# WangChangqi98/CSS

Hardware: AMD Instinct MI355X
Metric: training images/sec at 513x513 R101-DeepLabv3+ (mix_label step, labeled+unlabeled crops consumed) (higher is better)
Workload: dtype bf16

## Files before the change

css_amd/csrc/abi.hip:

```cpp
#include "../../include/css_hip.h"
#include "launchers.h"

#include <cstdlib>
#include <cstring>
#include <mutex>
#include <new>
#include <vector>

namespace {
inline hipStream_t S(css_stream_t s) { return reinterpret_cast<hipStream_t>(s); }
inline void set_dev(int device) {
  if (device >= 0) (void)hipSetDevice(device);
}
int g_cu_count[64] = {0};
int cu_count(int device) {
  int d = device;
  if (d < 0) (void)hipGetDevice(&d);
  if (d < 0 || d >= 64) return 256;
  if (!g_cu_count[d]) {
    int v = 0;
    if (hipDeviceGetAttribute(&v, hipDeviceAttributeMultiprocessorCount, d) != hipSuccess || v <= 0) v = 256;
    g_cu_count[d] = v;
  }
  return g_cu_count[d];
// ... 117 lines not shown
int css_conv2d_forward_bnstats(const void* x, const void* w, void* y, float* stats, int Mg, int N, int H, int W, int Cin, int ldx, int Ho, int Wo,
                               int Cout, int ldy, int R, int Sk, int stride, int pad, int dil, double alg_flops, int dtype, int device,
                               css_stream_t stream) {
  set_dev(device);
  ConvArgs a = {};
  a.src = x; a.wt = w; a.dst = y; a.bias = nullptr;
  a.N = N; a.Hs = H; a.Ws = W; a.Cs = Cin; a.lds = ldx;
  a.Hd = Ho; a.Wd = Wo; a.Cd = Cout; a.ldd = ldy;
  a.R = R; a.S = Sk; a.stride = stride; a.pad = pad; a.dil = dil; a.mode = 0;
  a.M = N * Ho * Wo; a.Ktot = R * Sk * Cin;
  a.stats = stats; a.stat_Mg = Mg;
  if (!stats || Mg < 128 || a.M % Mg) return CSS_ERR_ARG;
  ConvProf cp(0, 5, alg_flops, S(stream));
  cp.hbm_bytes = short_k_bytes(a, dtype);
  cp.ws_bytes = conv1x1_bytes(a, dtype);
  cp.conv_bytes = conv_alg_bytes(a, dtype);
  return css_launch_conv(a, dtype, cu_count(device), S(stream), g_prof_on ? &cp : nullptr);
}
int css_conv2d_forward_bnstats_tile_rows(const void* x, const void* w, void* y, int N, int H, int W, int Cin, int ldx, int Ho, int Wo, int Cout,
                                         int ldy, int R, int Sk, int stride, int pad, int dil, int dtype, int device) {
  ConvArgs a = {};
  a.src = x; a.wt = w; a.dst = y; a.bias = nullptr;
  a.N = N; a.Hs = H; a.Ws = W; a.Cs = Cin; a.lds = ldx;
  a.Hd = Ho; a.Wd = Wo; a.Cd = Cout; a.ldd = ldy;
  a.R = R; a.S = Sk; a.stride = stride; a.pad = pad; a.dil = dil; a.mode = 0;
  a.M = N * Ho * Wo; a.Ktot = R * Sk * Cin;
  alignas(16) static float dummy[4];
  a.stats = dummy; a.stat_Mg = a.M;
  return css_conv_tile_rows_(a, dtype, cu_count(device));
}
int css_conv2d_dgrad(const void* dy, const void* w_t, void* dx, int N, int H, int W, int Cin, int lddx, int Ho, int Wo, int Cout, int lddy, int R,
                     int Sk, int stride, int pad, int dil, double alg_flops, int dtype, int device, css_stream_t stream) {
  set_dev(device);
  if (stride != 1 && stride != 2) return CSS_ERR_ARG;
  ConvArgs a = {};
  a.src = dy; a.wt = w_t; a.dst = dx; a.bias = nullptr;
  a.N = N; a.Hs = Ho; a.Ws = Wo; a.Cs = Cout; a.lds = lddy;
  a.Hd = H; a.Wd = W; a.Cd = Cin; a.ldd = lddx;
  a.R = R; a.S = Sk; a.stride = stride; a.pad = pad; a.dil = dil; a.mode = 1;
  a.M = N * H * W; a.Ktot = R * Sk * Cout;
  ConvProf cp(1, 6, alg_flops, S(stream));
  cp.ws_bytes = conv1x1_bytes(a, dtype);
  cp.conv_bytes = conv_alg_bytes(a, dtype);
  return css_launch_conv(a, dtype, cu_count(device), S(stream), g_prof_on ? &cp : nullptr);
}
static int dgrad_add_impl(const void* dy, const void* w_t, void* dx, const void* addend, int ld_add, const unsigned char* mask, int N, int H, int W, int Cin,
                          int lddx, int Ho, int Wo, int Cout, int lddy, int R, int Sk, int stride, int pad, int dil, double alg_flops, int dtype,
                          int device, css_stream_t stream) {
  set_dev(device);
  if (stride != 1 && stride != 2) return CSS_ERR_ARG;
  if (mask) {
    const int vec = dtype == CSS_BF16 ? 8 : 4;
    if (!addend || (Cin % vec) || (lddx % vec) || (ld_add % vec) || (reinterpret_cast<uintptr_t>(dx) & 15) || (reinterpret_cast<uintptr_t>(addend) & 15))
      return CSS_ERR_ARG;
  }
  ConvArgs a = {};
  a.src = dy; a.wt = w_t; a.dst = dx; a.bias = nullptr;
  a.N = N; a.Hs = Ho; a.Ws = Wo; a.Cs = Cout; a.lds = lddy;
  a.Hd = H; a.Wd = W; a.Cd = Cin; a.ldd = lddx;
  a.R = R; a.S = Sk; a.stride = stride; a.pad = pad; a.dil = dil; a.mode = 1; a.addend = addend; a.ld_add = ld_add; a.add_mask = mask;
  a.M = N * H * W; a.Ktot = R * Sk * Cout;
  ConvProf cp(1, 6, alg_flops, S(stream));
  cp.ws_bytes = conv1x1_bytes(a, dtype);
  cp.conv_bytes = conv_alg_bytes(a, dtype);
  return css_launch_conv(a, dtype, cu_count(device), S(stream), g_prof_on ? &cp : nullptr);
}
int css_conv2d_dgrad_add(const void* dy, const void* w_t, void* dx, const void* addend, int ld_add, int N, int H, int W, int Cin, int lddx, int Ho, int Wo, int Cout, int lddy, int R,
                     int Sk, int stride, int pad, int dil, double alg_flops, int dtype, int device, css_stream_t stream) {
  return dgrad_add_impl(dy, w_t, dx, addend, ld_add, nullptr, N, H, W, Cin, lddx, Ho, Wo, Cout, lddy, R, Sk, stride, pad, dil, alg_flops, dtype, device, stream);
}
int css_conv2d_dgrad_add_masked(const void* dy, const void* w_t, void* dx, const void* addend, int ld_add, const unsigned char* mask, int N, int H, int W, int Cin,
                                int lddx, int Ho, int Wo, int Cout, int lddy, int R, int Sk, int stride, int pad, int dil, double alg_flops, int dtype,
                                int device, css_stream_t stream) {
  if (!mask) return CSS_ERR_ARG;
  return dgrad_add_impl(dy, w_t, dx, addend, ld_add, mask, N, H, W, Cin, lddx, Ho, Wo, Cout, lddy, R, Sk, stride, pad, dil, alg_flops, dtype, device, stream);
}
size_t css_conv2d_wgrad_ws_bytes(int M, int Ktot, int Cout, int dtype, int device) {
  return css_wgrad_ws_bytes_(M, Ktot, Cout, dtype, cu_count(device));
}
int css_conv2d_wgrad(const void* x, const void* dy, float* dw, float* ws, size_t ws_bytes, int N, int H, int W, int Cin, int ldx, int Ho, int Wo,
                     int Cout, int lddy, int R, int Sk, int stride, int pad, int dil, double alg_flops, int dtype, int device,
                     css_stream_t stream) {
  set_dev(device);
  WgradArgs a;
  a.ws = ws; a.ws_bytes = ws ? ws_bytes : 0;
  a.x = x; a.dy = dy; a.dw = dw;
  a.N = N; a.Hs = H; a.Ws = W; a.Cs = Cin; a.ldx = ldx;
  a.Hd = Ho; a.Wd = Wo; a.Cd = Cout; a.ldy = lddy;
  a.R = R; a.S = Sk; a.stride = stride; a.pad = pad; a.dil = dil;
  a.M = N * Ho * Wo; a.Ktot = R * Sk * Cin; a.m_per_split = a.M;
  ConvProf cp(2, 7, alg_flops, S(stream));
  return css_launch_wgrad(a, dtype, cu_count(device), S(stream), g_prof_on ? &cp : nullptr);
}
int css_conv_ws_applies(int M, int K, int ld_src, int N, int ld_dst, int R, int Sk, int stride, int pad, int has_stats, int has_addend, int ld_add,
                        int has_bias, int dtype, int n_cu) {
  static const bool no_dma = getenv("CSS_NO_DMA_CONV") != nullptr, no_256 = getenv("CSS_NO_DMA256_CONV") != nullptr;
  if (dtype != CSS_BF16 || no_dma || no_256) return 0;
  alignas(16) static float dummy[4];
  ConvArgs a = {};
  a.N = 1; a.Hs = a.Hd = 1; a.Ws = a.Wd = M; a.M = M;
  a.Cs = K; a.lds = ld_src; a.Cd = N; a.ldd = ld_dst; a.Ktot = R * Sk * K;
  a.R = R; a.S = Sk; a.stride = stride; a.pad = pad; a.dil = 1;
  a.stats = has_stats ? dummy : nullptr;
  a.addend = has_addend ? dummy : nullptr; a.ld_add = ld_add;
  a.bias = has_bias ? dummy : nullptr;
  return css_conv_ws_supported(a, n_cu > 0 ? n_cu : 256) ? 1 : 0;
}
int css_conv_c64_applies(int N, int H, int W, int Cin, int ld_src, int Cout, int ld_dst, int R, int Sk, int stride, int pad, int dil, int has_addend,
                         int has_bias, int dtype) {
  static const bool no_dma = getenv("CSS_NO_DMA_CONV") != nullptr;
  if (no_dma) return 0;
  alignas(16) static float dummy[4];
  ConvArgs a = {};
  a.N = N; a.Hs = a.Hd = H; a.Ws = a.Wd = W; a.M = N * H * W;
  a.Cs = Cin; a.lds = ld_src; a.Cd = Cout; a.ldd = ld_dst; a.Ktot = R * Sk * Cin;
  a.R = R; a.S = Sk; a.stride = stride; a.pad = pad; a.dil = dil;
  a.src = a.wt = dummy; a.dst = dummy;
  a.addend = has_addend ? dummy : nullptr;
  a.bias = has_bias ? dummy : nullptr;
  return css_conv_c64_supported(a, dtype) ? 1 : 0;
}
int css_conv_c64_set_enabled(int on) { return css_conv_c64_set_enabled_(on); }
int css_wgrad_splits(int M, int Ktot, int Cout, int dtype, int n_cu) {
  int splits = 0, mps = 0;
  css_wgrad_plan_(M, Ktot, Cout, dtype, n_cu > 0 ? n_cu : 256, &splits, &mps);
  return splits;
}
int css_weight_layout(const float* w, void* out, int Cout, int taps, int Cin, int CinPad, int dgrad, int dtype, int device, css_stream_t stream) {
  set_dev(device);
  return css_launch_weight_layout(w, out, Cout, taps, Cin, CinPad, dgrad, dtype, S(stream));
}

int css_weight_dgrad_layout_batched(const float* flat, void* out, const long* desc, int n_layers, long total_tiles, int dtype, int device,
                                    css_stream_t stream) {
  set_dev(device);
  return css_launch_weight_dgrad_layout_batched(flat, out, desc, n_layers, total_tiles, dtype, S(stream));
}

int css_bn_nrb(int Mg, int G, int C, int dtype) { return css_bn_nrb_(Mg, G, C, dtype); }
int css_bn_stats(const void* y, int Mg, int G, int C, int ld, double* partial, int dtype, int device, css_stream_t stream) {
  set_dev(device);
  return css_launch_bn_stats(y, Mg, G, C, ld, partial, dtype, S(stream));
}
int css_bn_reduce(const double* partial, int nrb, int C, int G, double* sums, float* dgamma, float* dbeta, int accumulate, double count_local,
                  int device, css_stream_t stream) {
  set_dev(device);
  return css_launch_bn_reduce(partial, nrb, C, G, sums, dgamma, dbeta, accumulate, count_local, S(stream));
}
int css_bn_reduce_finalize(const double* partial, int nrb, int G, double count, const float* gamma, const float* beta, float* running_mean,
                           float* running_var, float momentum, float eps, float* mean, float* invstd, float* scale, float* shift, int C,
                           int device, css_stream_t stream) {
  set_dev(device);
  return css_launch_bn_reduce_finalize(partial, nrb, G, count, gamma, beta, running_mean, running_var, momentum, eps, mean, invstd, scale, shift,
                                       C, S(stream));
}
int css_bn_reduce_finalize_slabs(const float* partial, int M, int Mg, int G, double count, const float* gamma, const float* beta,
                                 float* running_mean, float* running_var, float momentum, float eps, float* mean, float* invstd, float* scale,
                                 float* shift, double* sums_out, int C, const void* y, int ldy, int tile_rows, int device, css_stream_t stream) {
  set_dev(device);
  return css_launch_bn_reduce_slabs(partial, M, Mg, G, count, gamma, beta, running_mean, running_var, momentum, eps, mean, invstd, scale, shift,
                                    sums_out, C, y, ldy, tile_rows, S(stream));
}
int css_bn_finalize(const double* sums, int G, double count, const double* count_dev, const float* gamma, const float* beta, float* running_mean,
                    float* running_var, float momentum, float eps, float* mean, float* invstd, float* scale, float* shift, int C, int device,
                    css_stream_t stream) {
  set_dev(device);
  return css_launch_bn_finalize(sums, G, count, count_dev, gamma, beta, running_mean, running_var, momentum, eps, mean, invstd, scale, shift, C, S(stream));
// ... 324 lines not shown
```

css_amd/csrc/bn.hip:

```cpp
#include "common.h"
#include <type_traits>
#include <cstdlib>

template <typename T, typename F>
__device__ __forceinline__ void channel_reduce2(F f, int Mg, int C, int rows_per_block, double* partial, bool rev = false) {
  constexpr int VEC = 16 / sizeof(T);
  const int CV = C / VEC;
  const int TPC = CV < 256 ? CV : 256;
  const int RPB = 256 / TPC;
  const int tid = threadIdx.x;
  const int cvi = tid % TPC, rg = tid / TPC;
  const int cv = blockIdx.y * TPC + cvi;
  const bool active = rg < RPB && cv < CV;
  float s0[VEC], s1[VEC];
#pragma unroll
  for (int e = 0; e < VEC; ++e) s0[e] = s1[e] = 0.f;
  const int gbase = blockIdx.z * Mg;
  const int bx = rev ? (int)(gridDim.x - 1 - blockIdx.x) : (int)blockIdx.x;
  const int row0 = gbase + bx * rows_per_block;
  const int row1 = min(gbase + Mg, row0 + rows_per_block);
  if (active) {
    int r = row0 + rg;
    for (; r + 3 * RPB < row1; r += 4 * RPB) {
      f(r, cv * VEC, s0, s1);
// ... 138 lines not shown
  shift_out[c] = bet - fmean * sc;
  if (running_mean) {
    const double unbiased = count > 1 ? var * count / (count - 1) : var;
    rm = (1.f - momentum) * rm + momentum * fmean;
    rv = (1.f - momentum) * rv + momentum * (float)unbiased;
    running_mean[c] = rm;
    running_var[c] = rv;
  }
}
__global__ __launch_bounds__(1024) void bn_reduce_kernel(const double* __restrict__ partial, int nrb, int C, int G, double* __restrict__ sums,
                                                         float* __restrict__ g1, float* __restrict__ g0, int accumulate, double count_local) {
  double t0 = 0, t1 = 0;
  if (sums && count_local > 0 && blockIdx.x == 0 && threadIdx.x < G) sums[(size_t)G * 2 * C + threadIdx.x] = count_local;
  const int ce = blockIdx.x * S2_CH + (int)threadIdx.x;
  float old0 = 0.f, old1 = 0.f;
  if (accumulate && g0 && threadIdx.x < S2_CH && ce < C) { old0 = g0[ce]; old1 = g1[ce]; }
  stage2_reduce(
      partial, C, G, [&](int g, int& lo, int& hi) { lo = g * nrb; hi = lo + nrb; },
      [&](int g, double a0, double a1, int c) {
        if (sums) { sums[(size_t)g * 2 * C + c] = a0; sums[(size_t)g * 2 * C + C + c] = a1; }
        t0 += a0; t1 += a1;
        if (g == G - 1 && g0) {
          g0[c] = old0 + (float)t0;
          g1[c] = old1 + (float)t1;
        }
      });
}
__global__ __launch_bounds__(1024) void bn_reduce_finalize_kernel(const double* __restrict__ partial, int nrb, int G, double count,
                                                                  const float* __restrict__ gamma, const float* __restrict__ beta,
                                                                  float* running_mean, float* running_var, float momentum, float eps,
                                                                  float* mean_out, float* invstd_out, float* scale_out, float* shift_out, int C) {
  const int ce = blockIdx.x * S2_CH + (int)threadIdx.x;
  float gam = 0.f, bet = 0.f, rm = 0.f, rv = 0.f;
  if (threadIdx.x < S2_CH && ce < C) {
    gam = gamma[ce]; bet = beta[ce];
    if (running_mean) { rm = running_mean[ce]; rv = running_var[ce]; }
  }
  stage2_reduce(
      partial, C, G, [&](int g, int& lo, int& hi) { lo = g * nrb; hi = lo + nrb; },
      [&](int g, double a0, double a1, int c) {
        bn_finalize_reg(a0, a1, count, gam, bet, rm, rv, running_mean, running_var, momentum, eps, mean_out + g * C, invstd_out + g * C,
                        scale_out + g * C, shift_out + g * C, c);
      });
}

__device__ __forceinline__ int slab_start(int p, int BM) { return (p >> 1) * BM + (p & 1) * (BM - 128); }
__device__ __forceinline__ int first_slab_from(int row, int BM) {
  const int t = BM == 256 ? row >> 8 : row / BM, rem = row - t * BM;
  return 2 * t + (rem == 0 ? 0 : (rem <= BM - 128 ? 1 : 2));
}
__global__ __launch_bounds__(1024) void bn_reduce_slabs_kernel(const float* __restrict__ partial, int nslab, int Mg, int G, double count,
                                                               const float* __restrict__ gamma, const float* __restrict__ beta,
                                                               float* running_mean, float* running_var, float momentum, float eps,
                                                               float* mean_out, float* invstd_out, float* scale_out, float* shift_out,
                                                               double* sums_out, int C, const bf16_t* __restrict__ y, int ldy, int BM) {
  if (sums_out && blockIdx.x == 0 && threadIdx.x < G) sums_out[(size_t)G * 2 * C + threadIdx.x] = (double)Mg;
  const int ce = blockIdx.x * S2_CH + (int)threadIdx.x;
  float gam = 0.f, bet = 0.f, rm = 0.f, rv = 0.f;
  if (!sums_out && threadIdx.x < S2_CH && ce < C) {
    gam = gamma[ce]; bet = beta[ce];
    if (running_mean) { rm = running_mean[ce]; rv = running_var[ce]; }
  }
  stage2_reduce(
      partial, C, G,
      [&](int g, int& lo, int& hi) {
        const int b = g * Mg, e = b + Mg;
        lo = first_slab_from(b, BM);
        hi = first_slab_from(e, BM);
        if (hi > nslab) hi = nslab;
      },
      [&](int g, double a0, double a1, int c) {
        if (sums_out) {
          sums_out[(size_t)g * 2 * C + c] = a0;
          sums_out[(size_t)g * 2 * C + C + c] = a1;
        } else {
          bn_finalize_reg(a0, a1, count, gam, bet, rm, rv, running_mean, running_var, momentum, eps, mean_out + g * C, invstd_out + g * C,
                          scale_out + g * C, shift_out + g * C, c);
        }
      },
      [&](int g, int c, int pl, int P, double& t0, double& t1) {
        const int b = g * Mg;
        int e = slab_start(first_slab_from(b, BM), BM);
        if (e > b + Mg) e = b + Mg;
        for (int r = b + pl; r < e; r += P) {
          const float v = (float)y[(size_t)r * ldy + c];
          t0 += (double)v;
          t1 += (double)v * (double)v;
        }
      });
}

template <typename T>
__global__ __launch_bounds__(256) void bn_stats_kernel(const T* __restrict__ y, int Mg, int C, int ld,
                                                       int rows_per_block, double* partial) {
  constexpr int VEC = 16 / sizeof(T);
  auto f = [&](int r, int c, float* s0, float* s1) {
    Vec16<T> v;
    v.load(y + (size_t)r * ld + c);
#pragma unroll
    for (int e = 0; e < VEC; ++e) {
      float x = v.f(e);
      s0[e] += x;
      s1[e] += x * x;
    }
  };
  channel_reduce2<T>(f, Mg, C, rows_per_block, partial);
}

__global__ void bn_finalize_kernel(const double* __restrict__ sums, int G, double count, const double* __restrict__ count_dev,
                                   const float* __restrict__ gamma, const float* __restrict__ beta,
                                   float* running_mean, float* running_var, float momentum, float eps,
                                   float* mean_out, float* invstd_out, float* scale_out, float* shift_out, int C) {
  int c = blockIdx.x * blockDim.x + threadIdx.x;
  if (c >= C) return;
  for (int g = 0; g < G; ++g)
    bn_finalize_one(sums[(size_t)g * 2 * C + c], sums[(size_t)g * 2 * C + C + c], count_dev ? count_dev[g] : count, gamma[c], beta[c], running_mean, running_var, momentum, eps,
                    mean_out + g * C, invstd_out + g * C, scale_out + g * C, shift_out + g * C, c);
}

__global__ void bn_eval_coeff_kernel(const float* __restrict__ gamma, const float* __restrict__ beta,
                                     const float* __restrict__ running_mean, const float* __restrict__ running_var,
                                     float eps, float* scale_out, float* shift_out, int C) {
  int c = blockIdx.x * blockDim.x + threadIdx.x;
  if (c >= C) return;
  float invstd = 1.0f / sqrtf(running_var[c] + eps);
  float sc = gamma[c] * invstd;
  scale_out[c] = sc;
  shift_out[c] = beta[c] - running_mean[c] * sc;
}

#define EW_UNROLL 4
template <typename T, bool MASK, bool RES, bool RELU>
__global__ __launch_bounds__(256) void bn_apply_kernel(const T* __restrict__ y, int ldy, const T* __restrict__ res, int ldr,
                                                       T* __restrict__ out, int ldo, const float* __restrict__ scale,
                                                       const float* __restrict__ shift, int Mg, int C, int rows_per_block,
                                                       unsigned char* __restrict__ mask, int rev) {
  constexpr int VEC = 16 / sizeof(T);
  const int CV = C / VEC;
  const int TPC = CV < 256 ? CV : 256, RPB = 256 / TPC;
  const int cvi = threadIdx.x % TPC, rg = threadIdx.x / TPC;
  const int cv = blockIdx.y * TPC + cvi;
  if (rg >= RPB || cv >= CV) return;
  const int c = cv * VEC, g = blockIdx.z;
  using P = Pairs<T>;
  f32x2 sc[P::NP], sh[P::NP];
#pragma unroll
  for (int p = 0; p < P::NP; ++p) {
    sc[p] = f32x2{scale[g * C + c + 2 * p], scale[g * C + c + 2 * p + 1]};
    sh[p] = f32x2{shift[g * C + c + 2 * p], shift[g * C + c + 2 * p + 1]};
  }
  const int gbase = g * Mg;
  const int nt = rev >> 1;
  rev &= 1;
  const int bx = rev ? (int)(gridDim.x - 1 - blockIdx.x) : (int)blockIdx.x;
  const int row0 = gbase + bx * rows_per_block, row1 = min(gbase + Mg, row0 + rows_per_block);
  for (int r = row0 + rg; r < row1; r += EW_UNROLL * RPB) {
    Vec16<T> v[EW_UNROLL], rr[EW_UNROLL];
#pragma unroll
    for (int u = 0; u < EW_UNROLL; ++u) {
      const int ru = r + u * RPB;
      if (ru < row1) {
        v[u].load(y + (size_t)ru * ldy + c, (nt & 1) != 0);
        if (RES) rr[u].load(res + (size_t)ru * ldr + c, (nt & 2) != 0);
      }
    }
#pragma unroll
    for (int u = 0; u < EW_UNROLL; ++u) {
      const int ru = r + u * RPB;
      if (ru < row1) {
        Vec16<T> o;
#pragma unroll
// ... 435 lines not shown
```

css_amd/csrc/contrast.hip:

```cpp
#include "common.h"

constexpr int CT_MAXK = 32;
struct ContrastMeta {
  int V;
  int present[CT_MAXK];
  int cntV[CT_MAXK];
  int cntH[CT_MAXK];
  int baseV[CT_MAXK];
  int baseH[CT_MAXK];
  int err;
};

__global__ __launch_bounds__(256) void contrast_classify_kernel(const float* __restrict__ label, const float* __restrict__ mask,
                                                                const float* __restrict__ prob, long sb, long sk, long sp, long psb, long psk,
                                                                long psp, int P, int HW, int K, float strong_thr, int* __restrict__ cls,
                                                                uint8_t* __restrict__ hard, ContrastMeta* meta) {
  for (int p = blockIdx.x * blockDim.x + threadIdx.x; p < P; p += gridDim.x * blockDim.x) {
    const int b = p / HW, s = p - b * HW;
    const float m = mask[p];
    int c = -1, n = 0;
    for (int k = 0; k < K; ++k) {
      const float v = label[b * sb + k * sk + s * sp] * m;
      if (v != 0.f) { if (c < 0) c = k; ++n; }
    }
    if (n > 1) atomicOr(&meta->err, 1);
    cls[p] = c;
    hard[p] = (c >= 0 && prob[b * psb + c * psk + s * psp] < strong_thr) ? 1 : 0;
  }
}

template <typename T, int C>
__global__ __launch_bounds__(256) void contrast_class_sums_kernel(const T* __restrict__ rep, int ld, const int* __restrict__ cls, int P, int K,
                                                                  int pix_per_block, float* __restrict__ out) {
  extern __shared__ float cs_lds[];
  const int tid = threadIdx.x, lane = tid & 63, wave = tid >> 6;
  float* acc = cs_lds + (size_t)wave * K * C;
  float* cnt = cs_lds + (size_t)4 * K * C + wave * CT_MAXK;
  for (int i = lane; i < K * C; i += 64) acc[i] = 0.f;
  if (lane < CT_MAXK) cnt[lane] = 0.f;
  __syncthreads();
  const int p0 = blockIdx.x * pix_per_block, p1 = min(P, p0 + pix_per_block);
  constexpr int EPL = C / 64, UN = 16;
  static_assert(EPL == 4, "a lane owns one float4 of the accumulator row");
  int cur = -1;
  float racc[4] = {0.f, 0.f, 0.f, 0.f}, rcnt = 0.f;
  auto flush = [&]() {
    if (cur >= 0) {
      float4* a4 = reinterpret_cast<float4*>(acc + cur * C + lane * EPL);
      float4 a = *a4;
      a.x += racc[0]; a.y += racc[1]; a.z += racc[2]; a.w += racc[3];
      *a4 = a;
      if (lane == 0) cnt[cur] += rcnt;
    }
    racc[0] = racc[1] = racc[2] = racc[3] = 0.f;
    rcnt = 0.f;
  };
  for (int pb = p0 + wave * 64; pb < p1; pb += 4 * 64) {
    const int ci = pb + lane < p1 ? cls[pb + lane] : -1;
#pragma unroll
    for (int u0 = 0; u0 < 64; u0 += UN) {
      int c[UN];
      float v[UN][EPL];
#pragma unroll
      for (int u = 0; u < UN; ++u) c[u] = __builtin_amdgcn_readlane(ci, u0 + u);
#pragma unroll
      for (int u = 0; u < UN; ++u) {
        if (c[u] >= 0) {
          const T* row = rep + (size_t)(pb + u0 + u) * ld + lane * EPL;
          if constexpr (sizeof(T) == 2) {
            union { uint2 u2; T e[EPL]; } pk;
            pk.u2 = *reinterpret_cast<const uint2*>(row);
#pragma unroll
            for (int e = 0; e < EPL; ++e) v[u][e] = (float)pk.e[e];
          } else {
#pragma unroll
            for (int e = 0; e < EPL; ++e) v[u][e] = (float)row[e];
          }
        }
      }
#pragma unroll
      for (int u = 0; u < UN; ++u) {
        if (c[u] < 0) continue;
        if (c[u] != cur) {
          flush();
          cur = c[u];
        }
        racc[0] += v[u][0]; racc[1] += v[u][1]; racc[2] += v[u][2]; racc[3] += v[u][3];
        rcnt += 1.f;
      }
    }
  }
  flush();
  __syncthreads();
  float* row = out + (size_t)blockIdx.x * (K * C + K);
  for (int i = tid; i < K * C; i += 256)
    row[i] = (cs_lds[i] + cs_lds[(size_t)K * C + i]) + (cs_lds[(size_t)2 * K * C + i] + cs_lds[(size_t)3 * K * C + i]);
  if (tid < K) {
    const float* cb = cs_lds + (size_t)4 * K * C;
    row[(size_t)K * C + tid] = (cb[tid] + cb[CT_MAXK + tid]) + (cb[2 * CT_MAXK + tid] + cb[3 * CT_MAXK + tid]);
  }
}
__global__ __launch_bounds__(256) void contrast_class_sums_reduce_kernel(const float* __restrict__ ws, int nrows, int n, double* __restrict__ out) {
  const int i = blockIdx.x * 256 + threadIdx.x;
  if (i >= n) return;
  double s0 = 0, s1 = 0, s2 = 0, s3 = 0;
  int r = 0;
  for (; r + 3 < nrows; r += 4) {
    s0 += (double)ws[(size_t)(r + 0) * n + i]; s1 += (double)ws[(size_t)(r + 1) * n + i];
    s2 += (double)ws[(size_t)(r + 2) * n + i]; s3 += (double)ws[(size_t)(r + 3) * n + i];
  }
  for (; r < nrows; ++r) s0 += (double)ws[(size_t)r * n + i];
  out[i] = (s0 + s1) + (s2 + s3);
}

constexpr int CHUNK_R = 16;
__global__ __launch_bounds__(256) void contrast_hist_kernel(const int* __restrict__ cls, const uint8_t* __restrict__ hard, int P, int K,
                                                            int* __restrict__ chunkhist) {
  const int lane = threadIdx.x & 63;
  const int chunk = blockIdx.x * 4 + (threadIdx.x >> 6);
  const int p0 = chunk * 64 * CHUNK_R;
  if (p0 >= P) return;
  int mine = 0;
  for (int r = 0; r < CHUNK_R; ++r) {
    const int p = p0 + r * 64 + lane;
    const int c = p < P ? cls[p] : -1;
    const int h = (p < P && c >= 0) ? hard[p] : 0;
    for (int k = 0; k < K; ++k) {
      const unsigned long long bv = __ballot(c == k), bh = __ballot(c == k && h);
      if (lane == k) mine += __popcll(bv);
      if (lane == 32 + k) mine += __popcll(bh);
    }
  }
  chunkhist[chunk * 64 + lane] = mine;
}
__global__ __launch_bounds__(64) void contrast_scan_kernel(int* __restrict__ chunkhist, int nchunks, int K, ContrastMeta* meta) {
  const int t = threadIdx.x;
  int run = 0;
  constexpr int SCAN_U = 16;
  for (int c0 = 0; c0 < nchunks; c0 += SCAN_U) {
    int v[SCAN_U];
#pragma unroll
    for (int u = 0; u < SCAN_U; ++u) v[u] = c0 + u < nchunks ? chunkhist[(c0 + u) * 64 + t] : 0;
#pragma unroll
    for (int u = 0; u < SCAN_U; ++u) {
      if (c0 + u < nchunks) chunkhist[(c0 + u) * 64 + t] = run;
      run += v[u];
    }
  }
  __shared__ int tot[64];
  tot[t] = run;
  __syncthreads();
  if (t == 0) {
    int bv = 0, bh = 0, V = 0;
    for (int k = 0; k < CT_MAXK; ++k) {
      const int cv = k < K ? tot[k] : 0, ch = k < K ? tot[32 + k] : 0;
      meta->cntV[k] = cv;
      meta->cntH[k] = ch;
      meta->baseV[k] = bv;
      meta->baseH[k] = bh;
      bv += cv;
// ... 373 lines not shown
```

css_amd/csrc/conv_wgrad.hip:

```cpp
#include "common.h"
#include "launchers.h"
#include <cstdlib>


template <typename T> struct WgFrag;
template <> struct WgFrag<bf16_t> {
  static constexpr int KS = 16;
  typedef bf16x8 frag;
  static __device__ __forceinline__ frag load(const bf16_t* tile, int RS, int kk0, int col0, int lane) {
    const int i = lane & 15, g = lane >> 4, q = i >> 2, p = i & 3;
    const bf16_t* ad = tile + (kk0 + 8 * (g >> 1) + q) * RS + col0 + 16 * (g & 1) + 4 * p;
    typedef __attribute__((address_space(3))) s16x4 lds_v4;
    s16x4 lo = __builtin_amdgcn_ds_read_tr16_b64_v4i16((lds_v4*)(ad));
    s16x4 hi = __builtin_amdgcn_ds_read_tr16_b64_v4i16((lds_v4*)(ad + 4 * RS));
    union { struct { s16x4 a, b; } s; frag f; } u;
    u.s.a = lo;
    u.s.b = hi;
    return u.f;
  }
  static __device__ __forceinline__ f32x16 mma(frag a, frag b, f32x16 c) {
    return __builtin_amdgcn_mfma_f32_32x32x16_bf16(a, b, c, 0, 0, 0);
  }
};
template <> struct WgFrag<float> {
// ... 484 lines not shown
#pragma unroll
        for (int i = 0; i < 4; ++i) acc[j][i] = __builtin_amdgcn_mfma_f32_16x16x32_bf16(j < 2 ? cur[j] : fx23[j - 2], fy[i], acc[j][i], 0, 0, 0);
#pragma unroll
      for (int g_ = 0; g_ < 16; ++g_) {
        __builtin_amdgcn_sched_group_barrier(0x008, 1, 0);
        __builtin_amdgcn_sched_group_barrier(0x006, 2, 0);
      }
      __builtin_amdgcn_sched_barrier(0);
      __builtin_amdgcn_s_barrier();
      asm volatile("" ::: "memory");
      __builtin_amdgcn_sched_barrier(0);
#pragma unroll
      for (int i = 0; i < 4; ++i) fy[i] = frag(fad[4 + i]);
      nxt[0] = frag(fad[TN + 0] + dn);
      nxt[1] = frag(fad[TN + 1] + dn);
      __builtin_amdgcn_sched_barrier(0);
      stage_half(st_i, 1, vy, vx);
      asm volatile("s_waitcnt lgkmcnt(0)" ::: "memory");
      __builtin_amdgcn_sched_barrier(0);
      __builtin_amdgcn_s_barrier();
      __builtin_amdgcn_sched_barrier(0);
      row_offsets(0, vy, vx);
#pragma unroll
      for (int k = 4; k < TN + 2; ++k) {
        fad[k] += dn;
        asm volatile("" : "+v"(fad[k]));
      }
#pragma unroll
      for (int j = 0; j < TK; ++j)
#pragma unroll
        for (int i = 0; i < 4; ++i) acc[j][4 + i] = __builtin_amdgcn_mfma_f32_16x16x32_bf16(j < 2 ? cur[j] : fx23[j - 2], fy[i], acc[j][4 + i], 0, 0, 0);
#pragma unroll
      for (int g_ = 0; g_ < 16; ++g_) {
        __builtin_amdgcn_sched_group_barrier(0x008, 1, 0);
        __builtin_amdgcn_sched_group_barrier(0x006, 2, 0);
      }
      __builtin_amdgcn_sched_barrier(0);
      __builtin_amdgcn_s_barrier();
      asm volatile("" ::: "memory");
      __builtin_amdgcn_sched_barrier(0);
      st_c = st_c == NST - 1 ? 0 : st_c + 1;
      st_i = st_i == NST - 1 ? 0 : st_i + 1;
    };
    int it = 0;
    for (; it + 1 < nit; it += 2) {
      step(fxa, fxb);
      step(fxb, fxa);
    }
    if (it < nit) step(fxa, fxb);
    WG_STAMP_END();
    if (wn == 0) __builtin_amdgcn_s_barrier();
    asm volatile("s_waitcnt vmcnt(0)" ::: "memory");
    const int l15 = lane & 15, lg = lane >> 4;
    if (a.ws) {
      float* slab = a.ws + ((size_t)t * a.splits + zz) * (256 * 256);
#pragma unroll
      for (int i = 0; i < TN; ++i) {
        const int nl = wn * WTN + i * 16 + l15;
#pragma unroll
        for (int j = 0; j < TK; ++j) {
          const int kl = wk * WTK + j * 16 + 4 * lg;
          if (a.nt & 1) __builtin_nontemporal_store(acc[j][i], reinterpret_cast<f32x4*>(slab + nl * 256 + kl));
          else *reinterpret_cast<f32x4*>(slab + nl * 256 + kl) = acc[j][i];
        }
      }
      return;
    }
#pragma unroll
    for (int i = 0; i < TN; ++i) {
      const int n = n0 + wn * WTN + i * 16 + l15;
      if (n >= a.Cd) continue;
#pragma unroll
      for (int j = 0; j < TK; ++j)
#pragma unroll
        for (int r = 0; r < 4; ++r) {
          const int k = k0 + wk * WTK + j * 16 + 4 * lg + r;
          if (k < a.Ktot) atomicAdd(a.dw + (size_t)n * a.Ktot + k, acc[j][i][r]);
        }
    }
  }
}

typedef __attribute__((ext_vector_type(4))) float wg_f32x4;
__device__ __forceinline__ float4 wg_ld4(const float4* p, bool nt) {
  if (!nt) return *p;
  const wg_f32x4 t = __builtin_nontemporal_load(reinterpret_cast<const wg_f32x4*>(p));
  return make_float4(t[0], t[1], t[2], t[3]);
}
__global__ __launch_bounds__(256) void wgrad_slab_reduce_kernel(const float* __restrict__ ws, float* __restrict__ dw, int splits, int tiles_k,
                                                                int Cd, int Ktot, int nt) {
  const int t = blockIdx.y;
  const int k0 = (t % tiles_k) * 256, n0 = (t / tiles_k) * 256;
  const int nl = blockIdx.x * 4 + (threadIdx.x >> 6), kl = (threadIdx.x & 63) * 4;
  const int n = n0 + nl, k = k0 + kl;
  if (n >= Cd || k >= Ktot) return;
  const float4* p = reinterpret_cast<const float4*>(ws + (size_t)t * splits * (256 * 256) + nl * 256 + kl);
  float4 s0 = make_float4(0.f, 0.f, 0.f, 0.f), s1 = s0, s2 = s0, s3 = s0;
  int z = 0;
  for (; z + 3 < splits; z += 4) {
    const float4 v0 = wg_ld4(p + (size_t)(z + 0) * (256 * 256 / 4), nt), v1 = wg_ld4(p + (size_t)(z + 1) * (256 * 256 / 4), nt);
    const float4 v2 = wg_ld4(p + (size_t)(z + 2) * (256 * 256 / 4), nt), v3 = wg_ld4(p + (size_t)(z + 3) * (256 * 256 / 4), nt);
    s0.x += v0.x; s0.y += v0.y; s0.z += v0.z; s0.w += v0.w;
    s1.x += v1.x; s1.y += v1.y; s1.z += v1.z; s1.w += v1.w;
    s2.x += v2.x; s2.y += v2.y; s2.z += v2.z; s2.w += v2.w;
    s3.x += v3.x; s3.y += v3.y; s3.z += v3.z; s3.w += v3.w;
  }
  for (; z < splits; ++z) {
    const float4 v0 = wg_ld4(p + (size_t)z * (256 * 256 / 4), nt);
    s0.x += v0.x; s0.y += v0.y; s0.z += v0.z; s0.w += v0.w;
  }
  const float r[4] = {(s0.x + s1.x) + (s2.x + s3.x), (s0.y + s1.y) + (s2.y + s3.y), (s0.z + s1.z) + (s2.z + s3.z), (s0.w + s1.w) + (s2.w + s3.w)};
  float* o = dw + (size_t)n * Ktot + k;
#pragma unroll
  for (int e = 0; e < 4; ++e)
    if (k + e < Ktot) o[e] += r[e];
}

template <int BN_, int BKC>
__global__ __launch_bounds__(256) void wgrad_slab_reduce_gen_kernel(const float* __restrict__ ws, float* __restrict__ dw, int splits, int tiles_k,
                                                                    int Cd, int Ktot, int nt) {
  constexpr int TPR = BKC / 4, RPB = 256 / TPR;
  const int t = blockIdx.y;
  const int k0 = (t % tiles_k) * BKC, n0 = (t / tiles_k) * BN_;
  const int nl = blockIdx.x * RPB + threadIdx.x / TPR, kl = (threadIdx.x % TPR) * 4;
  const int n = n0 + nl, k = k0 + kl;
  if (nl >= BN_ || n >= Cd || k >= Ktot) return;
  const float4* p = reinterpret_cast<const float4*>(ws + (size_t)t * splits * (BN_ * BKC) + nl * BKC + kl);
  constexpr size_t SL = (size_t)BN_ * BKC / 4;
  float4 s0 = make_float4(0.f, 0.f, 0.f, 0.f), s1 = s0, s2 = s0, s3 = s0;
  int z = 0;
  for (; z + 3 < splits; z += 4) {
    const float4 v0 = wg_ld4(p + (size_t)(z + 0) * SL, nt), v1 = wg_ld4(p + (size_t)(z + 1) * SL, nt), v2 = wg_ld4(p + (size_t)(z + 2) * SL, nt),
                 v3 = wg_ld4(p + (size_t)(z + 3) * SL, nt);
    s0.x += v0.x; s0.y += v0.y; s0.z += v0.z; s0.w += v0.w;
    s1.x += v1.x; s1.y += v1.y; s1.z += v1.z; s1.w += v1.w;
    s2.x += v2.x; s2.y += v2.y; s2.z += v2.z; s2.w += v2.w;
    s3.x += v3.x; s3.y += v3.y; s3.z += v3.z; s3.w += v3.w;
  }
  for (; z < splits; ++z) {
    const float4 v0 = wg_ld4(p + (size_t)z * SL, nt);
    s0.x += v0.x; s0.y += v0.y; s0.z += v0.z; s0.w += v0.w;
  }
  const float r[4] = {(s0.x + s1.x) + (s2.x + s3.x), (s0.y + s1.y) + (s2.y + s3.y), (s0.z + s1.z) + (s2.z + s3.z), (s0.w + s1.w) + (s2.w + s3.w)};
  float* o = dw + (size_t)n * Ktot + k;
#pragma unroll
  for (int e = 0; e < 4; ++e)
    if (k + e < Ktot) o[e] += r[e];
}


static bool wgrad_n64(int dtype, int Cd, bool big) {
  static const bool on = getenv("CSS_WGRAD_N64") && atoi(getenv("CSS_WGRAD_N64")) != 0;
  return on && dtype == CSS_BF16 && !big && Cd <= 64;
}
void css_wgrad_plan_(int M, int Ktot, int Cd, int dtype, int n_cu, int* splits_out, int* mps_out) {
  static const bool no_256 = getenv("CSS_NO_DMA256_WGRAD") != nullptr;
  const bool big = dtype == CSS_BF16 && Cd >= 256 && Ktot >= 256 && !no_256;
  const bool n64 = wgrad_n64(dtype, Cd, big);
  const int bn = dtype == CSS_BF16 ? (big ? 256 : (n64 ? 64 : 128)) : 64, bkc = bn, bp = dtype == CSS_BF16 ? (big ? 32 : 64) : 16;
  const int tiles = cdiv(Ktot, bkc) * cdiv(Cd, bn);
  const int places = n_cu * (big ? 1 : (n64 ? 3 : 2));
  const double t_step = big ? 0.86 : (dtype == CSS_BF16 ? 1.1 : 1.0), t_fix = big ? 5.0 : 3.0;
  const double t_slab = (double)bn * bkc * 4 * 2 / 4.0e6;
  int best_s = 1;
  double best = 1e300;
  for (int s = 1; s <= 1024; ++s) {
    const int mps = cdiv(cdiv(M, s), bp) * bp;
    if (s > 1 && mps < 4 * bp) break;
    if (cdiv(M, mps) != s) continue;
    const double rounds = (double)cdiv((long)tiles * s, places);
    const double cost = rounds * ((double)(mps / bp) * t_step + t_fix) + (double)tiles * s * t_slab;
    if (cost < best - 1e-9) { best = cost; best_s = s; }
  }
  const int mps = cdiv(cdiv(M, best_s), bp) * bp;
  *splits_out = cdiv(M, mps);
  *mps_out = mps;
}

size_t css_wgrad_ws_bytes_(int M, int Ktot, int Cd, int dtype, int n_cu) {
  static const bool no_256 = getenv("CSS_NO_DMA256_WGRAD") != nullptr, no_ws = getenv("CSS_WGRAD_ATOMICS") != nullptr;
  if (no_ws || M <= 0 || (dtype != CSS_BF16 && dtype != CSS_F32)) return 0;
  int splits, mps;
  css_wgrad_plan_(M, Ktot, Cd, dtype, n_cu, &splits, &mps);
  const bool big = dtype == CSS_BF16 && Cd >= 256 && Ktot >= 256 && !no_256;
  const int bn = big ? 256 : (dtype == CSS_BF16 && !wgrad_n64(dtype, Cd, big) ? 128 : 64);
  return (size_t)cdiv(Ktot, bn) * cdiv(Cd, bn) * splits * ((size_t)bn * bn * sizeof(float));
}

int css_wgrad_mfma_override_ = 0;
int css_wgrad_no_compact_override_ = 0;
int css_launch_wgrad(WgradArgs a, int dtype, int n_cu, hipStream_t st, LaunchProf* prof) {
  if (a.M <= 0) return CSS_OK;
  a.fd_hw = make_fastdiv((uint32_t)(a.Hd * a.Wd));
  a.fd_w = make_fastdiv((uint32_t)a.Wd);
  int bn, bkc, bp;
  static const bool no_256 = getenv("CSS_NO_DMA256_WGRAD") != nullptr;
  const bool big = dtype == CSS_BF16 && a.Cd >= 256 && a.Ktot >= 256 && !no_256;
  const bool n64 = wgrad_n64(dtype, a.Cd, big);
  if (dtype == CSS_BF16) {
    bn = big ? 256 : (n64 ? 64 : 128); bkc = bn; bp = big ? 32 : 64;
    if (a.Cs % 8 || a.ldx % 8 || a.ldy % 8 || a.Cd % 8) return CSS_ERR_ARG;
  } else if (dtype == CSS_F32) {
    bn = 64; bkc = 64; bp = 16;
    if (a.Cs % 4 || a.ldx % 4 || a.ldy % 4 || a.Cd % 4) return CSS_ERR_ARG;
  } else {
    return CSS_ERR_DTYPE;
  }
  if ((reinterpret_cast<uintptr_t>(a.x) & 15) || (reinterpret_cast<uintptr_t>(a.dy) & 15)) return CSS_ERR_ARG;
  {
    const size_t esz = dtype == CSS_BF16 ? 2 : 4;
    const size_t xb = (size_t)a.N * a.Hs * a.Ws * a.ldx * esz, yb = (size_t)a.M * a.ldy * esz;
    if (xb >= 0x7FFFFFF0ull || yb >= 0x7FFFFFF0ull) return CSS_ERR_ARG;
    a.x_bytes = (unsigned)xb;
    a.dy_bytes = (unsigned)yb;
  }
  int splits, mps;
  css_wgrad_plan_(a.M, a.Ktot, a.Cd, dtype, n_cu, &splits, &mps);
  a.m_per_split = mps;
  a.splits = splits;
  a.tiles_k = cdiv(a.Ktot, bkc);
  a.tiles_n = cdiv(a.Cd, bn);
  static const int wg_nt = getenv("CSS_WGRAD_NT") ? atoi(getenv("CSS_WGRAD_NT")) & 3 : 2;
  a.nt = wg_nt & 1;
  const int rnt = (wg_nt >> 1) & 1;
  a.compact = 0;
  {
    static const bool no_compact = getenv("CSS_WGRAD_NO_COMPACT") && atoi(getenv("CSS_WGRAD_NO_COMPACT")) != 0;
    if (big && !no_compact && !css_wgrad_no_compact_override_ && a.R > 1 && a.R <= 3 && a.stride == 1 && a.Cs % 256 == 0) {
      bool any = false;
      for (int r = 0; r < a.R; ++r) {
        const int dh = r * a.dil - a.pad;
        int lo = dh < 0 ? -dh : 0, hi = a.Hd - 1 < a.Hs - 1 - dh ? a.Hd - 1 : a.Hs - 1 - dh;
        if (hi < lo) { lo = 0; hi = a.Hd - 1; }
        a.row_lo[r] = lo;
        a.row_n[r] = hi - lo + 1;
        a.row_mps[r] = cdiv(cdiv(a.N * a.row_n[r] * a.Wd, splits), bp) * bp;
        a.fd_L[r] = make_fastdiv((uint32_t)(a.row_n[r] * a.Wd));
        any = any || a.row_n[r] < a.Hd;
      }
      a.compact = any ? 1 : 0;
      static const bool no_lpt = getenv("CSS_WGRAD_NO_LONGEST_FIRST") && atoi(getenv("CSS_WGRAD_NO_LONGEST_FIRST")) != 0;
      if (any && !no_lpt && a.tiles_k % a.R == 0) {
        a.cls_nrows[0] = a.cls_nrows[1] = 0;
        for (int r = 0; r < a.R; ++r) {
          const int c = a.row_n[r] == a.Hd ? 0 : 1;
          a.cls_rows[c][a.cls_nrows[c]++] = r;
        }
        if (a.cls_nrows[0] > 0 && a.cls_nrows[1] > 0) a.compact = 2;
      }
    }
  }
  dim3 g(cdiv((long)a.tiles_k * a.tiles_n * splits, 8) * 8);
  if (a.compact == 2) {
    const int tpr = a.tiles_k / a.R;
    g = dim3(8 * (cdiv(a.tiles_n * a.cls_nrows[0] * tpr * splits, 8) + cdiv(a.tiles_n * a.cls_nrows[1] * tpr * splits, 8)));
  }
  if (prof) prof->begin(big, 1.0, false);
  if ((size_t)a.tiles_k * a.tiles_n * a.splits * ((size_t)bn * bkc * sizeof(float)) > a.ws_bytes) a.ws = nullptr;
  if (big) {
    static const bool env16 = getenv("CSS_WGRAD_MFMA") && atoi(getenv("CSS_WGRAD_MFMA")) == 16;
    const bool mf16 = css_wgrad_mfma_override_ ? css_wgrad_mfma_override_ == 16 : env16;
    if (mf16) hipLaunchKernelGGL(conv_wgrad_p8_kernel<true>, g, dim3(512), 0, st, a);
    else hipLaunchKernelGGL(conv_wgrad_p8_kernel<false>, g, dim3(512), 0, st, a);
    if (a.ws)
      hipLaunchKernelGGL(wgrad_slab_reduce_kernel, dim3(64, a.tiles_k * a.tiles_n), dim3(256), 0, st, a.ws, a.dw, a.splits, a.tiles_k, a.Cd, a.Ktot, rnt);
  } else if (n64) {
    hipLaunchKernelGGL((conv_wgrad_kernel<bf16_t, 64, 64, 64>), g, dim3(256), 0, st, a);
    if (a.ws)
      hipLaunchKernelGGL((wgrad_slab_reduce_gen_kernel<64, 64>), dim3(64 / 16, a.tiles_k * a.tiles_n), dim3(256), 0, st, a.ws, a.dw, a.splits,
                         a.tiles_k, a.Cd, a.Ktot, rnt);
  } else if (dtype == CSS_BF16) {
    hipLaunchKernelGGL((conv_wgrad_kernel<bf16_t, 128, 128, 64>), g, dim3(256), 0, st, a);
    if (a.ws)
      hipLaunchKernelGGL((wgrad_slab_reduce_gen_kernel<128, 128>), dim3(128 / 8, a.tiles_k * a.tiles_n), dim3(256), 0, st, a.ws, a.dw, a.splits,
                         a.tiles_k, a.Cd, a.Ktot, rnt);
  } else {
    hipLaunchKernelGGL((conv_wgrad_kernel<float, 64, 64, 16>), g, dim3(256), 0, st, a);
    if (a.ws)
      hipLaunchKernelGGL((wgrad_slab_reduce_gen_kernel<64, 64>), dim3(64 / 16, a.tiles_k * a.tiles_n), dim3(256), 0, st, a.ws, a.dw, a.splits,
                         a.tiles_k, a.Cd, a.Ktot, rnt);
  }
  if (prof) prof->end();
  CSS_CHECK_LAUNCH();
  return CSS_OK;
}
```

Before: 299.7.

## Raise memory-level parallelism in wgrad slab reduce, BN tail stats, and contrast gather

Rewrites the wgrad split-K slab reduction to issue sixteen loads per iteration, pinned with asm barriers, and adds a vectorised float4 read-modify-write of dw when it is aligned. It also limits waves per EU through an occupancy attribute, and the four reduce launches now share one dispatcher. The BN stats tail loop becomes a fixed-count predicated gather, and the contrast kernel prefetches the next class indices and issues all row loads unconditionally before converting them. Together these aim to hide memory latency in reduction and gather loops, at the cost of more registers and some redundant loads of clamped rows.

```diff
diff --git a/css_amd/csrc/abi.hip b/css_amd/csrc/abi.hip
--- a/css_amd/csrc/abi.hip
+++ b/css_amd/csrc/abi.hip
@@ -223,7 +223,7 @@
                      int Cout, int lddy, int R, int Sk, int stride, int pad, int dil, double alg_flops, int dtype, int device,
                      css_stream_t stream) {
   set_dev(device);
-  WgradArgs a;
+  WgradArgs a = {};
   a.ws = ws; a.ws_bytes = ws ? ws_bytes : 0;
   a.x = x; a.dy = dy; a.dw = dw;
   a.N = N; a.Hs = H; a.Ws = W; a.Cs = Cin; a.ldx = ldx;
diff --git a/css_amd/csrc/bn.hip b/css_amd/csrc/bn.hip
--- a/css_amd/csrc/bn.hip
+++ b/css_amd/csrc/bn.hip
@@ -244,11 +244,22 @@
         const int b = g * Mg;
         int e = slab_start(first_slab_from(b, BM), BM);
         if (e > b + Mg) e = b + Mg;
-        for (int r = b + pl; r < e; r += P) {
-          const float v = (float)y[(size_t)r * ldy + c];
-          t0 += (double)v;
-          t1 += (double)v * (double)v;
-        }
+        const int n = e - b;
+        auto head = [&](auto uc) {
+          constexpr int U = decltype(uc)::value;
+          bf16_t v[U];
+#pragma unroll
+          for (int u = 0; u < U; ++u) v[u] = y[(size_t)(b + (pl + u * P < n ? pl + u * P : 0)) * ldy + c];
+#pragma unroll
+          for (int u = 0; u < U; ++u) {
+            const double x = (double)(float)v[u];
+            const bool ok = pl + u * P < n;
+            t0 = ok ? t0 + x : t0;
+            t1 = ok ? t1 + x * x : t1;
+          }
+        };
+        if (n > 4 * P) head(std::integral_constant<int, 16>());
+        else if (n > 0) head(std::integral_constant<int, 4>());
       });
 }
 
diff --git a/css_amd/csrc/contrast.hip b/css_amd/csrc/contrast.hip
--- a/css_amd/csrc/contrast.hip
+++ b/css_amd/csrc/contrast.hip
@@ -1,4 +1,5 @@
 #include "common.h"
+#include <type_traits>
 
 constexpr int CT_MAXK = 32;
 struct ContrastMeta {
@@ -55,27 +56,34 @@
     racc[0] = racc[1] = racc[2] = racc[3] = 0.f;
     rcnt = 0.f;
   };
+  using Raw = typename std::conditional<sizeof(T) == 2, uint2, float4>::type;
+  int ci_next = p0 + wave * 64 + lane < p1 ? cls[p0 + wave * 64 + lane] : -1;
   for (int pb = p0 + wave * 64; pb < p1; pb += 4 * 64) {
-    const int ci = pb + lane < p1 ? cls[pb + lane] : -1;
+    const int ci = ci_next;
+    ci_next = pb + 4 * 64 + lane < p1 ? cls[pb + 4 * 64 + lane] : -1;
 #pragma unroll
     for (int u0 = 0; u0 < 64; u0 += UN) {
       int c[UN];
+      Raw raw[UN];
       float v[UN][EPL];
 #pragma unroll
       for (int u = 0; u < UN; ++u) c[u] = __builtin_amdgcn_readlane(ci, u0 + u);
 #pragma unroll
       for (int u = 0; u < UN; ++u) {
-        if (c[u] >= 0) {
-          const T* row = rep + (size_t)(pb + u0 + u) * ld + lane * EPL;
-          if constexpr (sizeof(T) == 2) {
-            union { uint2 u2; T e[EPL]; } pk;
-            pk.u2 = *reinterpret_cast<const uint2*>(row);
-#pragma unroll
-            for (int e = 0; e < EPL; ++e) v[u][e] = (float)pk.e[e];
-          } else {
-#pragma unroll
-            for (int e = 0; e < EPL; ++e) v[u][e] = (float)row[e];
-          }
+        const int pr = c[u] >= 0 ? pb + u0 + u : p0;
+        raw[u] = *reinterpret_cast<const Raw*>(rep + (size_t)pr * ld + lane * EPL);
+      }
+#pragma unroll
+      for (int u = 0; u < UN; ++u) {
+        if constexpr (sizeof(T) == 2) {
+          asm volatile("" : "+v"(raw[u].x), "+v"(raw[u].y));
+          union { uint2 u2; T e[EPL]; } pk;
+          pk.u2 = raw[u];
+#pragma unroll
+          for (int e = 0; e < EPL; ++e) v[u][e] = (float)pk.e[e];
+        } else {
+          asm volatile("" : "+v"(raw[u].x), "+v"(raw[u].y), "+v"(raw[u].z), "+v"(raw[u].w));
+          v[u][0] = raw[u].x; v[u][1] = raw[u].y; v[u][2] = raw[u].z; v[u][3] = raw[u].w;
         }
       }
 #pragma unroll
diff --git a/css_amd/csrc/conv_wgrad.hip b/css_amd/csrc/conv_wgrad.hip
--- a/css_amd/csrc/conv_wgrad.hip
+++ b/css_amd/csrc/conv_wgrad.hip
@@ -590,43 +590,78 @@
 }
 
 typedef __attribute__((ext_vector_type(4))) float wg_f32x4;
-__device__ __forceinline__ float4 wg_ld4(const float4* p, bool nt) {
-  if (!nt) return *p;
-  const wg_f32x4 t = __builtin_nontemporal_load(reinterpret_cast<const wg_f32x4*>(p));
-  return make_float4(t[0], t[1], t[2], t[3]);
-}
-__global__ __launch_bounds__(256) void wgrad_slab_reduce_kernel(const float* __restrict__ ws, float* __restrict__ dw, int splits, int tiles_k,
-                                                                int Cd, int Ktot, int nt) {
+constexpr int WG_RED_U = 16;
+#define WG_RED_OCC __attribute__((amdgpu_waves_per_eu(1, 4)))
+#define WG_PIN15(v)                                                                                                                           \
+  "+v"(v[0]), "+v"(v[1]), "+v"(v[2]), "+v"(v[3]), "+v"(v[4]), "+v"(v[5]), "+v"(v[6]), "+v"(v[7]), "+v"(v[8]), "+v"(v[9]), "+v"(v[10]), "+v"(v[11]), \
+      "+v"(v[12]), "+v"(v[13]), "+v"(v[14])
+template <bool NT>
+__device__ __forceinline__ wg_f32x4 wg_ld4(const float4* p) {
+  if constexpr (NT) return __builtin_nontemporal_load(reinterpret_cast<const wg_f32x4*>(p));
+  else return *reinterpret_cast<const wg_f32x4*>(p);
+}
+template <bool NT, bool V4>
+__device__ __forceinline__ void wg_slab_reduce_thread(const float4* __restrict__ p, size_t SL, int splits, float* __restrict__ o, int kleft) {
+  wg_f32x4 old;
+  if constexpr (V4) {
+    old = *reinterpret_cast<const wg_f32x4*>(o);
+  } else {
+    old[0] = o[0]; old[1] = o[kleft > 1 ? 1 : 0]; old[2] = o[kleft > 2 ? 2 : 0]; old[3] = o[kleft > 3 ? 3 : 0];
+  }
+  wg_f32x4 s0 = {0.f, 0.f, 0.f, 0.f}, s1 = s0, s2 = s0, s3 = s0;
+  const int z4 = splits & ~3;
+  int z = 0;
+  for (; z + WG_RED_U <= splits; z += WG_RED_U) {
+    wg_f32x4 v[WG_RED_U];
+#pragma unroll
+    for (int u = 0; u < WG_RED_U; ++u) v[u] = wg_ld4<NT>(p + (size_t)(z + u) * SL);
+    asm volatile("" : WG_PIN15(v), "+v"(v[15]));
+    s0 += v[0]; s1 += v[1]; s2 += v[2]; s3 += v[3];
+    s0 += v[4]; s1 += v[5]; s2 += v[6]; s3 += v[7];
+    s0 += v[8]; s1 += v[9]; s2 += v[10]; s3 += v[11];
+    s0 += v[12]; s1 += v[13]; s2 += v[14]; s3 += v[15];
+  }
+  if (z < splits) {
+    wg_f32x4 v[WG_RED_U - 1];
+#pragma unroll
+    for (int u = 0; u < WG_RED_U - 1; ++u) v[u] = wg_ld4<NT>(p + (size_t)(z + u < splits ? z + u : splits - 1) * SL);
+    asm volatile("" : WG_PIN15(v));
+#pragma unroll
+    for (int u = 0; u < WG_RED_U - 1; u += 4) {
+      const bool ok0 = z + u < splits, ok1 = z + u + 1 < splits, ok2 = z + u + 2 < splits, tail = z + u >= z4;
+      s0 = ok0 ? s0 + v[u] : s0;
+      s0 = ok1 && tail ? s0 + v[u + 1] : s0;
+      s1 = ok1 && !tail ? s1 + v[u + 1] : s1;
+      s0 = ok2 && tail ? s0 + v[u + 2] : s0;
+      s2 = ok2 && !tail ? s2 + v[u + 2] : s2;
+      if (u + 3 < WG_RED_U - 1) s3 = !tail ? s3 + v[u + 3] : s3;
+    }
+  }
+  const wg_f32x4 r = old + ((s0 + s1) + (s2 + s3));
+  if constexpr (V4) {
+    *reinterpret_cast<wg_f32x4*>(o) = r;
+  } else {
+    o[0] = r[0];
+    if (kleft > 1) o[1] = r[1];
+    if (kleft > 2) o[2] = r[2];
+    if (kleft > 3) o[3] = r[3];
+  }
+}
+template <bool NT, bool V4>
+__global__ __launch_bounds__(256) WG_RED_OCC void wgrad_slab_reduce_kernel(const float* __restrict__ ws, float* __restrict__ dw, int splits, int tiles_k,
+                                                                int Cd, int Ktot) {
   const int t = blockIdx.y;
   const int k0 = (t % tiles_k) * 256, n0 = (t / tiles_k) * 256;
   const int nl = blockIdx.x * 4 + (threadIdx.x >> 6), kl = (threadIdx.x & 63) * 4;
   const int n = n0 + nl, k = k0 + kl;
   if (n >= Cd || k >= Ktot) return;
   const float4* p = reinterpret_cast<const float4*>(ws + (size_t)t * splits * (256 * 256) + nl * 256 + kl);
-  float4 s0 = make_float4(0.f, 0.f, 0.f, 0.f), s1 = s0, s2 = s0, s3 = s0;
-  int z = 0;
-  for (; z + 3 < splits; z += 4) {
-    const float4 v0 = wg_ld4(p + (size_t)(z + 0) * (256 * 256 / 4), nt), v1 = wg_ld4(p + (size_t)(z + 1) * (256 * 256 / 4), nt);
-    const float4 v2 = wg_ld4(p + (size_t)(z + 2) * (256 * 256 / 4), nt), v3 = wg_ld4(p + (size_t)(z + 3) * (256 * 256 / 4), nt);
-    s0.x += v0.x; s0.y += v0.y; s0.z += v0.z; s0.w += v0.w;
-    s1.x += v1.x; s1.y += v1.y; s1.z += v1.z; s1.w += v1.w;
-    s2.x += v2.x; s2.y += v2.y; s2.z += v2.z; s2.w += v2.w;
-    s3.x += v3.x; s3.y += v3.y; s3.z += v3.z; s3.w += v3.w;
-  }
-  for (; z < splits; ++z) {
-    const float4 v0 = wg_ld4(p + (size_t)z * (256 * 256 / 4), nt);
-    s0.x += v0.x; s0.y += v0.y; s0.z += v0.z; s0.w += v0.w;
-  }
-  const float r[4] = {(s0.x + s1.x) + (s2.x + s3.x), (s0.y + s1.y) + (s2.y + s3.y), (s0.z + s1.z) + (s2.z + s3.z), (s0.w + s1.w) + (s2.w + s3.w)};
-  float* o = dw + (size_t)n * Ktot + k;
-#pragma unroll
-  for (int e = 0; e < 4; ++e)
-    if (k + e < Ktot) o[e] += r[e];
-}
-
-template <int BN_, int BKC>
-__global__ __launch_bounds__(256) void wgrad_slab_reduce_gen_kernel(const float* __restrict__ ws, float* __restrict__ dw, int splits, int tiles_k,
-                                                                    int Cd, int Ktot, int nt) {
+  wg_slab_reduce_thread<NT, V4>(p, 256 * 256 / 4, splits, dw + (size_t)n * Ktot + k, Ktot - k);
+}
+
+template <int BN_, int BKC, bool NT, bool V4>
+__global__ __launch_bounds__(256) WG_RED_OCC void wgrad_slab_reduce_gen_kernel(const float* __restrict__ ws, float* __restrict__ dw, int splits, int tiles_k,
+                                                                    int Cd, int Ktot) {
   constexpr int TPR = BKC / 4, RPB = 256 / TPR;
   const int t = blockIdx.y;
   const int k0 = (t % tiles_k) * BKC, n0 = (t / tiles_k) * BN_;
@@ -634,28 +669,22 @@
   const int n = n0 + nl, k = k0 + kl;
   if (nl >= BN_ || n >= Cd || k >= Ktot) return;
   const float4* p = reinterpret_cast<const float4*>(ws + (size_t)t * splits * (BN_ * BKC) + nl * BKC + kl);
-  constexpr size_t SL = (size_t)BN_ * BKC / 4;
-  float4 s0 = make_float4(0.f, 0.f, 0.f, 0.f), s1 = s0, s2 = s0, s3 = s0;
-  int z = 0;
-  for (; z + 3 < splits; z += 4) {
-    const float4 v0 = wg_ld4(p + (size_t)(z + 0) * SL, nt), v1 = wg_ld4(p + (size_t)(z + 1) * SL, nt), v2 = wg_ld4(p + (size_t)(z + 2) * SL, nt),
-                 v3 = wg_ld4(p + (size_t)(z + 3) * SL, nt);
-    s0.x += v0.x; s0.y += v0.y; s0.z += v0.z; s0.w += v0.w;
-    s1.x += v1.x; s1.y += v1.y; s1.z += v1.z; s1.w += v1.w;
-    s2.x += v2.x; s2.y += v2.y; s2.z += v2.z; s2.w += v2.w;
-    s3.x += v3.x; s3.y += v3.y; s3.z += v3.z; s3.w += v3.w;
-  }
-  for (; z < splits; ++z) {
-    const float4 v0 = wg_ld4(p + (size_t)z * SL, nt);
-    s0.x += v0.x; s0.y += v0.y; s0.z += v0.z; s0.w += v0.w;
-  }
-  const float r[4] = {(s0.x + s1.x) + (s2.x + s3.x), (s0.y + s1.y) + (s2.y + s3.y), (s0.z + s1.z) + (s2.z + s3.z), (s0.w + s1.w) + (s2.w + s3.w)};
-  float* o = dw + (size_t)n * Ktot + k;
-#pragma unroll
-  for (int e = 0; e < 4; ++e)
-    if (k + e < Ktot) o[e] += r[e];
-}
-
+  wg_slab_reduce_thread<NT, V4>(p, (size_t)BN_ * BKC / 4, splits, dw + (size_t)n * Ktot + k, Ktot - k);
+}
+template <bool NT, bool V4>
+static void wg_launch_reduce_(int bn, int tiles, hipStream_t st, const float* ws, float* dw, int splits, int tiles_k, int Cd, int Ktot) {
+  const dim3 g(bn * bn / 1024, tiles);
+  if (bn == 256) hipLaunchKernelGGL((wgrad_slab_reduce_kernel<NT, V4>), g, dim3(256), 0, st, ws, dw, splits, tiles_k, Cd, Ktot);
+  else if (bn == 128) hipLaunchKernelGGL((wgrad_slab_reduce_gen_kernel<128, 128, NT, V4>), g, dim3(256), 0, st, ws, dw, splits, tiles_k, Cd, Ktot);
+  else hipLaunchKernelGGL((wgrad_slab_reduce_gen_kernel<64, 64, NT, V4>), g, dim3(256), 0, st, ws, dw, splits, tiles_k, Cd, Ktot);
+}
+static void wg_launch_reduce(bool nt, int bn, int tiles, hipStream_t st, const float* ws, float* dw, int splits, int tiles_k, int Cd, int Ktot) {
+  const bool v4 = (reinterpret_cast<uintptr_t>(dw) & 15) == 0 && Ktot % 4 == 0;
+  if (nt) v4 ? wg_launch_reduce_<true, true>(bn, tiles, st, ws, dw, splits, tiles_k, Cd, Ktot)
+             : wg_launch_reduce_<true, false>(bn, tiles, st, ws, dw, splits, tiles_k, Cd, Ktot);
+  else v4 ? wg_launch_reduce_<false, true>(bn, tiles, st, ws, dw, splits, tiles_k, Cd, Ktot)
+          : wg_launch_reduce_<false, false>(bn, tiles, st, ws, dw, splits, tiles_k, Cd, Ktot);
+}
 
 static bool wgrad_n64(int dtype, int Cd, bool big) {
   static const bool on = getenv("CSS_WGRAD_N64") && atoi(getenv("CSS_WGRAD_N64")) != 0;
@@ -770,24 +799,14 @@
     const bool mf16 = css_wgrad_mfma_override_ ? css_wgrad_mfma_override_ == 16 : env16;
     if (mf16) hipLaunchKernelGGL(conv_wgrad_p8_kernel<true>, g, dim3(512), 0, st, a);
     else hipLaunchKernelGGL(conv_wgrad_p8_kernel<false>, g, dim3(512), 0, st, a);
-    if (a.ws)
-      hipLaunchKernelGGL(wgrad_slab_reduce_kernel, dim3(64, a.tiles_k * a.tiles_n), dim3(256), 0, st, a.ws, a.dw, a.splits, a.tiles_k, a.Cd, a.Ktot, rnt);
   } else if (n64) {
     hipLaunchKernelGGL((conv_wgrad_kernel<bf16_t, 64, 64, 64>), g, dim3(256), 0, st, a);
-    if (a.ws)
-      hipLaunchKernelGGL((wgrad_slab_reduce_gen_kernel<64, 64>), dim3(64 / 16, a.tiles_k * a.tiles_n), dim3(256), 0, st, a.ws, a.dw, a.splits,
-                         a.tiles_k, a.Cd, a.Ktot, rnt);
   } else if (dtype == CSS_BF16) {
     hipLaunchKernelGGL((conv_wgrad_kernel<bf16_t, 128, 128, 64>), g, dim3(256), 0, st, a);
-    if (a.ws)
-      hipLaunchKernelGGL((wgrad_slab_reduce_gen_kernel<128, 128>), dim3(128 / 8, a.tiles_k * a.tiles_n), dim3(256), 0, st, a.ws, a.dw, a.splits,
-                         a.tiles_k, a.Cd, a.Ktot, rnt);
   } else {
     hipLaunchKernelGGL((conv_wgrad_kernel<float, 64, 64, 16>), g, dim3(256), 0, st, a);
-    if (a.ws)
-      hipLaunchKernelGGL((wgrad_slab_reduce_gen_kernel<64, 64>), dim3(64 / 16, a.tiles_k * a.tiles_n), dim3(256), 0, st, a.ws, a.dw, a.splits,
-                         a.tiles_k, a.Cd, a.Ktot, rnt);
-  }
+  }
+  if (a.ws) wg_launch_reduce(rnt != 0, bn, a.tiles_k * a.tiles_n, st, a.ws, a.dw, a.splits, a.tiles_k, a.Cd, a.Ktot);
   if (prof) prof->end();
   CSS_CHECK_LAUNCH();
   return CSS_OK;
```

After: 302.3, median of 6. About the same (+0.9%).
